# tuplex/tuplex

Measured on AMD Instinct MI355X. Metric: rows/s, higher is better.
Workload: dtype u8; 1 GPU; zillow-Z1 csv->map/withColumn/filter->tocsv (BASELINE.json configs[1]); mb_per_gpu=1024, sink=csv-device-resident

## Files before the change

### tuplex_amd/csrc/tpx_ci.hip.h

```cpp

#define TPX_CI_BYTES 4096
#define TPX_CI_RF_OFF 0
#define TPX_CI_BAD_OFF 136
#define TPX_CI_ENT_OFF 264
#define TPX_CI_CAP ((TPX_CI_BYTES - TPX_CI_ENT_OFF) / 4)
#define TPX_CI_NONE 0xFFFFu

__device__ __forceinline__ unsigned tpx_ci_zero32(unsigned x) {
    return ~(x | ((x | 0x80808080u) - 0x01010101u)) & 0x80808080u;
}

__device__ __forceinline__ unsigned tpx_ci_pack4(unsigned h) {
    unsigned x = h >> 7;
    x |= x >> 7;
    x |= x >> 14;
    return x & 0xFu;
}

struct tpx_ci_cls { unsigned q, s, n, r, h; };

__device__ __forceinline__ void tpx_ci_classify(unsigned w0, unsigned w1,
                                                unsigned w2, unsigned w3,
                                                char delim, unsigned valid,
                                                tpx_ci_cls* c) {
    const unsigned one = 0x01010101u;
    unsigned pq = one * (unsigned)'"', pd = one * (unsigned char)delim;
    unsigned pn = one * (unsigned)'\n', pr = one * (unsigned)'\r';
    unsigned w[4] = {w0, w1, w2, w3};
    unsigned q = 0, s = 0, n = 0, r = 0, h = 0;
    #pragma unroll
    for (int d = 0; d < 4; ++d) {
        unsigned v = w[d];
        unsigned zn = tpx_ci_zero32(v ^ pn);
        q |= tpx_ci_pack4(tpx_ci_zero32(v ^ pq)) << (4 * d);
        s |= tpx_ci_pack4(tpx_ci_zero32(v ^ pd) | zn) << (4 * d);
        n |= tpx_ci_pack4(zn) << (4 * d);
        r |= tpx_ci_pack4(tpx_ci_zero32(v ^ pr)) << (4 * d);
        h |= tpx_ci_pack4(v & 0x80808080u) << (4 * d);
    }
    c->q = q & valid; c->s = s & valid; c->n = n & valid;
    c->r = r & valid; c->h = h & valid;
}

__device__ __forceinline__ unsigned tpx_ci_inq(unsigned q16, unsigned par) {
    unsigned x = q16;
    x ^= x << 1; x ^= x << 2; x ^= x << 4; x ^= x << 8;
    x <<= 1;
    if (par) x = ~x;
    return x & 0xFFFFu;
}

__device__ __forceinline__ void tpx_ci_scatter(char* ci, int k, unsigned s16,
                                               unsigned n16, unsigned q16,
                                               unsigned ord, unsigned nl,
                                               unsigned qc0) {
    unsigned* ent = (unsigned*)(ci + TPX_CI_ENT_OFF);
    unsigned short* rf = (unsigned short*)(ci + TPX_CI_RF_OFF);
    while (s16) {
        int j = __ffs((int)s16) - 1;
        unsigned isnl = (n16 >> j) & 1u;
        unsigned qc = qc0 + (unsigned)__popc(q16 & ((1u << j) - 1u));
        if (ord < TPX_CI_CAP)
            ent[ord] = (unsigned)(k + j) | (isnl << 15) | (qc << 16);
        ++ord;
        if (isnl) {
            ++nl;
            if (nl <= 64 && ord <= TPX_CI_CAP) rf[nl] = (unsigned short)ord;
        }
        s16 &= s16 - 1;
    }
}

__device__ __forceinline__ int tpx_ci_row(const char* base, const char* ci,
                                          int r, int rs, int re, int rend,
                                          int span, int ncols, int* e0_out) {
    const unsigned* ent = (const unsigned*)(ci + TPX_CI_ENT_OFF);
    const unsigned short* rf = (const unsigned short*)(ci + TPX_CI_RF_OFF);
    const unsigned long long* bad =
        (const unsigned long long*)(ci + TPX_CI_BAD_OFF);
    if (re <= rs) return 0;
    unsigned e0 = rf[r], e1 = rf[r + 1];
    if (e0 == TPX_CI_NONE || e1 == TPX_CI_NONE) return 0;
    if (e1 != e0 + (unsigned)ncols) return 0;
    unsigned q = 0;
    if (e0 == 0) {
        if (r != 0) return 0;
    } else {
        unsigned pe = ent[e0 - 1];
        if (!(pe & 0x8000u) || (int)(pe & 0x3FFFu) != rs - 1) return 0;
        q = pe >> 16;
    }
    unsigned le = ent[e1 - 1];
    int lp = (int)(le & 0x3FFFu);
    if (le & 0x8000u) {
        if (lp != re - 1) return 0;
    } else {
        if (lp != re || re != span) return 0;
    }
    int b0 = rs >> 4, b1 = (re - 1) >> 4;
    for (int w = b0 >> 6; w <= (b1 >> 6); ++w) {
        int lo = w == (b0 >> 6) ? (b0 & 63) : 0;
        int hi = w == (b1 >> 6) ? (b1 & 63) : 63;
        unsigned long long m = (~0ULL << lo) & (~0ULL >> (63 - hi));
        if (bad[w] & m) return 0;
    }
    int cs = rs;
    for (int k = 0; k < ncols; ++k) {
        unsigned e = ent[e0 + (unsigned)k];
        int ce = k == ncols - 1 ? rend : (int)(e & 0x3FFFu);
        unsigned nq = ((e >> 16) - q) & 0xFFFFu;
        if (nq && (nq != 2 || ce - cs < 2 || base[cs] != '"' ||
                   base[ce - 1] != '"'))
            return 0;
        q = e >> 16;
        cs = (int)(e & 0x3FFFu) + 1;
    }
    *e0_out = (int)e0;
    return 1;
}

__device__ __forceinline__ void tpx_ci_cell(const char* base, const char* ci,
                                            int e0, int k, int ncols, int rs,
                                            int rend, tpx_cell* c) {
    const unsigned* ent = (const unsigned*)(ci + TPX_CI_ENT_OFF);
    unsigned e = ent[e0 + k];
    int cs = rs;
    unsigned q = 0;
    if (e0 + k > 0) {
        unsigned pe = ent[e0 + k - 1];
        cs = (int)(pe & 0x3FFFu) + 1;
        q = pe >> 16;
    }
    int ce = k == ncols - 1 ? rend : (int)(e & 0x3FFFu);
    if (((e >> 16) - q) & 0xFFFFu) {
        c->p = base + cs + 1; c->n = ce - cs - 2; c->flags = 1 | 8;
    } else {
        c->p = base + cs; c->n = ce - cs; c->flags = 0;
    }
}

#ifndef TPX_HOST_TEST
__device__ __forceinline__ unsigned tpx_wave_exscan32(unsigned v, int lane) {
    unsigned x = v;
    for (int o = 1; o < 64; o <<= 1) {
        unsigned y = __shfl_up(x, o);
        if (lane >= o) x += y;
    }
    return x - v;
}

__device__ __forceinline__ bool tpx_ci_stage(char* wave_lds, char* ci,
                                             const char* src, int span, int lo,
                                             char delim, int lane) {
    unsigned* ent = (unsigned*)(ci + TPX_CI_ENT_OFF);
    unsigned short* rf = (unsigned short*)(ci + TPX_CI_RF_OFF);
    unsigned long long* bad = (unsigned long long*)(ci + TPX_CI_BAD_OFF);
    rf[lane + 1] = (unsigned short)TPX_CI_NONE;
    if (lane == 0) rf[0] = 0;
    unsigned car_ord = 0, car_nl = 0, car_q = 0;
    bool pend = false;
    unsigned long long below = (1ull << lane) - 1ull;
    int trip = 0;
    uint4 pre = make_uint4(0, 0, 0, 0);
    if (lane * 16 + 16 <= span) pre = *(const uint4*)(src + lane * 16);
    for (int kb = 0; kb < span; kb += 64 * 16, ++trip) {
        int k = kb + lane * 16;
        unsigned w0 = 0, w1 = 0, w2 = 0, w3 = 0;
        if (k + 16 <= span) {
            uint4 v = pre;
            if (k + 64 * 16 + 16 <= span)
                pre = *(const uint4*)(src + k + 64 * 16);
            *(uint4*)(wave_lds + k) = v;
            w0 = v.x; w1 = v.y; w2 = v.z; w3 = v.w;
        } else {
            unsigned long long a = 0, b = 0;
            for (int j = k; j < span; ++j) {
                unsigned char ch = (unsigned char)src[j];
                wave_lds[j] = (char)ch;
                int t = j - k;
                if (t < 8) a |= (unsigned long long)ch << (8 * t);
                else b |= (unsigned long long)ch << (8 * (t - 8));
            }
            w0 = (unsigned)a; w1 = (unsigned)(a >> 32);
            w2 = (unsigned)b; w3 = (unsigned)(b >> 32);
        }
        int nv = span - k; nv = nv < 0 ? 0 : (nv > 16 ? 16 : nv);
        int nl_ = lo - k; nl_ = nl_ < 0 ? 0 : (nl_ > 16 ? 16 : nl_);
        unsigned valid = ((1u << nv) - 1u) & ~((1u << nl_) - 1u);
        tpx_ci_cls c;
        tpx_ci_classify(w0, w1, w2, w3, delim, valid, &c);
        unsigned pq = (unsigned)__popc(c.q);
        unsigned long long oddm = __ballot(pq & 1u);
        unsigned par = (car_q ^ (unsigned)__popcll(oddm & below)) & 1u;
        unsigned inq = tpx_ci_inq(c.q, par);
        unsigned s16 = c.s & ~inq, n16 = c.n & ~inq;
        unsigned ps = (unsigned)__popc(s16), pn = (unsigned)__popc(n16);
        unsigned ex = tpx_wave_exscan32(ps | (pn << 11) | (pq << 22), lane);
        unsigned xs = ex & 0x7FFu, xn = (ex >> 11) & 0x7FFu, xq = ex >> 22;
        unsigned long long nlf = __ballot(n16 & 1u);
        unsigned nxt = lane < 63 ? (unsigned)((nlf >> (lane + 1)) & 1ull) : 0u;
        unsigned badr = c.r & ~((n16 >> 1) | (nxt << 15));
        bool mypend = lane == 63 && (badr & 0x8000u);
        if (lane == 63) badr &= 0x7FFFu;
        unsigned long long bw = __ballot(c.h != 0 || badr != 0);
        if (lane == 0) {
            if (pend && !(nlf & 1ull)) bad[trip - 1] |= 1ull << 63;
            bad[trip] = bw;
        }
        pend = __ballot(mypend) != 0;
        tpx_ci_scatter(ci, k, s16, n16, c.q, car_ord + xs, car_nl + xn,
                       car_q + xq);
        car_ord += (unsigned)__builtin_amdgcn_readlane((int)(xs + ps), 63);
        car_nl += (unsigned)__builtin_amdgcn_readlane((int)(xn + pn), 63);
        car_q += (unsigned)__builtin_amdgcn_readlane((int)(xq + pq), 63);
    }
    if (pend && lane == 0) bad[trip - 1] |= 1ull << 63;
    bool ok = car_ord < TPX_CI_CAP;
    if (ok && car_nl < 64 && lane == 0) {
        ent[car_ord] = (unsigned)span | (car_q << 16);
        rf[car_nl + 1] = (unsigned short)(car_ord + 1);
    }
    __builtin_amdgcn_wave_barrier();
    return ok;
}
#endif
```

### tuplex_amd/csrc/tpx_rt.hip.h

```cpp
#pragma once
#if !defined(__HIPCC_RTC__) && !defined(__HIPRTC__)
#include <hip/hip_runtime.h>
#endif

#define TPX_WAVE 64

#ifndef TPX_OUTLINE
#define TPX_OUTLINE 0
#endif
#if TPX_OUTLINE
#define TPX_COLD __attribute__((noinline))
#else
#define TPX_COLD __forceinline__
#endif
#if TPX_OUTLINE >= 2
#define TPX_SHARED __attribute__((noinline))
#else
#define TPX_SHARED __forceinline__
#endif
struct tpx_i64r { long long v; int ec; };
struct tpx_f64r { double v; int ec; };

#define EC_OK 0
#define EC_NCV 7
// ... 639 lines not shown
    const char* p = start;
    bool neg = false;
    if (*p == '-') { neg = true; ++p; }
    while (p < end && *p >= '0' && *p <= '9') {
        x = x * 10 + (unsigned long long)(*p - '0');
        ++p;
    }
    if (p != end) return EC_I64PARSE;
    *out = (long long)(neg ? 0ULL - x : x);
    return EC_OK;
}

__device__ __forceinline__ int tpx_fast_atod(const char* start, const char* end,
                                             double* out) {
    if (start == end) return EC_NULLERROR;
    const char* p = start;
    double sign = 1.0;
    if (p < end && *p == '-') { sign = -1.0; ++p; }
    else if (p < end && *p == '+') ++p;
    double value = 0.0;
    while (p < end && *p >= '0' && *p <= '9') { value = 10.0 * value + (*p - '0'); ++p; }
    if (p < end && *p == '.') {
        double pow10 = 10.0;
        ++p;
        while (p < end && *p >= '0' && *p <= '9') {
            value += (*p - '0') / pow10;
            pow10 *= 10.0;
            ++p;
        }
    }
    int frac = 0;
    double scale = 1.0;
    if (p < end && (*p == 'e' || *p == 'E')) {
        ++p;
        if (p < end && *p == '-') { frac = 1; ++p; }
        else if (p < end && *p == '+') ++p;
        unsigned int exponent = 0;
        while (p < end && *p >= '0' && *p <= '9') { exponent = exponent * 10 + (*p - '0'); ++p; }
        if (exponent > 308) exponent = 308;
        while (exponent >= 50) { scale *= 1e50; exponent -= 50; }
        while (exponent >= 8)  { scale *= 1e8;  exponent -= 8; }
        while (exponent > 0)   { scale *= 10.0; exponent -= 1; }
    }
    int nanmatch = 0, infmatch = 0;
    if (p == start) {
        const char* t = "nan";
        while (nanmatch < 3 && p < end &&
               (*p == t[nanmatch] || *p == t[nanmatch] - 32)) { ++p; ++nanmatch; }
    }
    if (p == start) {
        const char* t = "infinity";
        while (infmatch < 8 && p < end &&
               (*p == t[infmatch] || *p == t[infmatch] - 32)) { ++p; ++infmatch; }
    }
    if (p != end) return EC_F64PARSE;
    if (nanmatch == 3) { *out = __builtin_nan(""); return EC_OK; }
    if (infmatch == 3 || infmatch == 8) { *out = sign * __builtin_inf(); return EC_OK; }
    *out = sign * (frac ? (value / scale) : (value * scale));
    return EC_OK;
}

__device__ TPX_SHARED tpx_i64r tpx_trim_atoi64(const char* p, long long n) {
    const char* a = p;
    const char* b = p + n;
    while (a < b && tpx_is_pyws(*a)) ++a;
    while (b > a && tpx_is_pyws(*(b - 1))) --b;
    tpx_i64r r{0, 0};
    r.ec = tpx_fast_atoi64(a, b, &r.v);
    return r;
}

__device__ TPX_SHARED tpx_f64r tpx_trim_atod(const char* p, long long n) {
    const char* a = p;
    const char* b = p + n;
    while (a < b && tpx_is_pyws(*a)) ++a;
    while (b > a && tpx_is_pyws(*(b - 1))) --b;
    tpx_f64r r{0.0, 0};
    r.ec = tpx_fast_atod(a, b, &r.v);
    return r;
}

__device__ __forceinline__ long long tpx_int_str(const tstr s, int* ec) {
    tpx_i64r r = tpx_trim_atoi64(s.p, s.n);
    if (r.ec != EC_OK) *ec = EC_VALUEERROR;
    return r.v;
}

__device__ __forceinline__ double tpx_float_str(const tstr s, int* ec) {
    tpx_f64r r = tpx_trim_atod(s.p, s.n);
    if (r.ec != EC_OK) *ec = EC_VALUEERROR;
    return r.v;
}

__device__ __forceinline__ long long tpx_int_f64(double x, int* ec) {
    if (!(x >= -9.223372036854775808e18 && x < 9.223372036854775808e18)) {
        *ec = x == x ? EC_OVERFLOW : EC_VALUEERROR;
        return 0;
    }
    return (long long)x;
}


__device__ __forceinline__ long long tpx_i64_digits(long long v) {
    unsigned long long x = v < 0 ? (unsigned long long)(-(v + 1)) + 1 : (unsigned long long)v;
    long long d = 1;
    while (x >= 10) { x /= 10; ++d; }
    return d + (v < 0 ? 1 : 0);
}

__device__ __forceinline__ void tpx_i64_write(char* dst, long long v, long long len) {
    unsigned long long x = v < 0 ? (unsigned long long)(-(v + 1)) + 1 : (unsigned long long)v;
    long long i = len;
    do { dst[--i] = '0' + (char)(x % 10); x /= 10; } while (x);
    if (v < 0) dst[0] = '-';
}

__device__ __forceinline__ tstr tpx_str_i64(TpxHeap& h, long long v, int* ec) {
    long long len = tpx_i64_digits(v);
    char* d = tpx_alloc(h, len);
    if (!d) { *ec = EC_MEMORYERROR; return tstr{nullptr, 0}; }
    tpx_i64_write(d, v, len);
    return tstr{d, len};
}

__device__ __forceinline__ tstr tpx_fmt0d(TpxHeap& h, long long width, long long v, int* ec) {
    long long dl = tpx_i64_digits(v);
    long long len = dl < width ? width : dl;
    char* d = tpx_alloc(h, len);
    if (!d) { *ec = EC_MEMORYERROR; return tstr{nullptr, 0}; }
    long long pad = len - dl;
    for (long long i = 0; i < pad; ++i) d[i] = '0';
    tpx_i64_write(d + pad, v, dl);
    if (v < 0 && pad > 0) {
        d[pad] = '0';
        d[0] = '-';
    }
    return tstr{d, len};
}

__device__ __forceinline__ tstr tpx_str_bool(bool b) {
    return b ? tstr{"True", 4} : tstr{"False", 5};
}

__device__ __forceinline__ tstr tpx_str_none() { return tstr{"None", 4}; }


__device__ TPX_SHARED long long tpx_csv_quote_scan(const tstr s) {
    bool need = false;
    long long q = 0;
    long long i = 0;
    while (i < s.n && (((unsigned long long)(s.p + i)) & 7)) {
        char c = s.p[i];
        if (c == '"') { ++q; need = true; }
        else if (c == ',' || c == '\n' || c == '\r') need = true;
        ++i;
    }
    for (; i + 32 <= s.n; i += 32) {
        unsigned long long v0 = *(const unsigned long long*)(s.p + i);
        unsigned long long v1 = *(const unsigned long long*)(s.p + i + 8);
        unsigned long long v2 = *(const unsigned long long*)(s.p + i + 16);
        unsigned long long v3 = *(const unsigned long long*)(s.p + i + 24);
        unsigned long long hq =
            tpx_swar_zero(v0 ^ (TPX_SWAR_ONE * (unsigned long long)'"')) |
            tpx_swar_zero(v1 ^ (TPX_SWAR_ONE * (unsigned long long)'"')) >> 1 |
            tpx_swar_zero(v2 ^ (TPX_SWAR_ONE * (unsigned long long)'"')) >> 2 |
            tpx_swar_zero(v3 ^ (TPX_SWAR_ONE * (unsigned long long)'"')) >> 3;
        unsigned long long ho = 0;
        ho |= tpx_swar_zero(v0 ^ (TPX_SWAR_ONE * (unsigned long long)',')) |
              tpx_swar_zero(v0 ^ (TPX_SWAR_ONE * (unsigned long long)'\n')) |
              tpx_swar_zero(v0 ^ (TPX_SWAR_ONE * (unsigned long long)'\r'));
        ho |= tpx_swar_zero(v1 ^ (TPX_SWAR_ONE * (unsigned long long)',')) |
              tpx_swar_zero(v1 ^ (TPX_SWAR_ONE * (unsigned long long)'\n')) |
              tpx_swar_zero(v1 ^ (TPX_SWAR_ONE * (unsigned long long)'\r'));
        ho |= tpx_swar_zero(v2 ^ (TPX_SWAR_ONE * (unsigned long long)',')) |
              tpx_swar_zero(v2 ^ (TPX_SWAR_ONE * (unsigned long long)'\n')) |
              tpx_swar_zero(v2 ^ (TPX_SWAR_ONE * (unsigned long long)'\r'));
        ho |= tpx_swar_zero(v3 ^ (TPX_SWAR_ONE * (unsigned long long)',')) |
              tpx_swar_zero(v3 ^ (TPX_SWAR_ONE * (unsigned long long)'\n')) |
              tpx_swar_zero(v3 ^ (TPX_SWAR_ONE * (unsigned long long)'\r'));
        if (hq) { q += __builtin_popcountll(hq); need = true; }
        if (ho) need = true;
    }
    for (; i + 8 <= s.n; i += 8) {
        unsigned long long v = *(const unsigned long long*)(s.p + i);
        unsigned long long hq =
            tpx_swar_zero(v ^ (TPX_SWAR_ONE * (unsigned long long)'"'));
        unsigned long long ho =
            tpx_swar_zero(v ^ (TPX_SWAR_ONE * (unsigned long long)',')) |
            tpx_swar_zero(v ^ (TPX_SWAR_ONE * (unsigned long long)'\n')) |
            tpx_swar_zero(v ^ (TPX_SWAR_ONE * (unsigned long long)'\r'));
        if (hq) { q += __builtin_popcountll(hq); need = true; }
        if (ho) need = true;
    }
    for (; i < s.n; ++i) {
        char c = s.p[i];
        if (c == '"') { ++q; need = true; }
        else if (c == ',' || c == '\n' || c == '\r') need = true;
    }
    return need ? q : -1;
}

__device__ __forceinline__ bool tpx_csv_needs_quote(const tstr s, long long* nquotes) {
    long long q = tpx_csv_quote_scan(s);
    *nquotes = q < 0 ? 0 : q;
    return q >= 0;
}

__device__ __forceinline__ long long tpx_csv_cell_len(const tstr s) {
    long long q;
    return tpx_csv_needs_quote(s, &q) ? s.n + q + 2 : s.n;
}

__device__ TPX_COLD char* tpx_csv_cell_write(char* w, const tstr s) {
    long long q;
    if (tpx_csv_needs_quote(s, &q)) {
        *w++ = '"';
        for (long long i = 0; i < s.n; ++i) {
            char c = s.p[i];
            *w++ = c;
            if (c == '"') *w++ = '"';
        }
        *w++ = '"';
    } else {
        tpx_memcpy(w, s.p, s.n);
        w += s.n;
    }
    return w;
}


struct tpx_f64n { unsigned long long N; int rc; bool neg; };

__device__ __forceinline__ int tpx_f64_csv_n_(double v, unsigned long long* N,
                                              bool* neg) {
    unsigned long long bits = (unsigned long long)__double_as_longlong(v);
    *neg = (bits >> 63) != 0;
    int exp = (int)((bits >> 52) & 0x7FF);
    unsigned long long man = bits & ((1ULL << 52) - 1);
    if (exp == 0x7FF) return 7;
    unsigned long long m;
    int e;
    if (exp == 0) { m = man; e = -1074; }
    else { m = man | (1ULL << 52); e = exp - 1075; }
    unsigned __int128 M = (unsigned __int128)m * 15625u;
    int k = e + 6;
    if (k >= 0) {
        if (k >= 62) return 7;
        unsigned __int128 S = M << k;
        if ((unsigned long long)(S >> 63)) return 7;
        *N = (unsigned long long)S;
        return 0;
    }
    k = -k;
    if (k >= 69) { *N = 0; return 0; }
    unsigned __int128 Nw = M >> k;
    unsigned __int128 rem = M & (((unsigned __int128)1 << k) - 1);
    unsigned __int128 half = (unsigned __int128)1 << (k - 1);
    if (rem > half || (rem == half && ((unsigned long long)Nw & 1))) ++Nw;
    if ((unsigned long long)(Nw >> 63)) return 7;
    *N = (unsigned long long)Nw;
    return 0;
}

__device__ TPX_SHARED tpx_f64n tpx_f64_csv_n_v(double v) {
    tpx_f64n r{0, 0, false};
    r.rc = tpx_f64_csv_n_(v, &r.N, &r.neg);
    return r;
}

__device__ __forceinline__ int tpx_f64_csv_n(double v, unsigned long long* N,
                                             bool* neg) {
    tpx_f64n r = tpx_f64_csv_n_v(v);
    if (r.rc == 0) *N = r.N;
    *neg = r.neg;
    return r.rc;
}

__device__ __forceinline__ long long tpx_f64_csv_len(unsigned long long N,
                                                     bool neg) {
    int d = 1;
    unsigned long long t = N;
    while (t >= 10) { t /= 10; ++d; }
    if (d < 7) d = 7;
    return (neg ? 1 : 0) + d + 1;
}

__device__ TPX_SHARED char* tpx_f64_csv_write(char* w,
                                            unsigned long long N,
                                            bool neg) {
    char buf[21];
    int nd = 0;
    unsigned long long t = N;
    do { buf[nd++] = (char)('0' + (t % 10)); t /= 10; } while (t);
    while (nd < 7) buf[nd++] = '0';
    if (neg) *w++ = '-';
    for (int i = nd - 1; i >= 6; --i) *w++ = buf[i];
    *w++ = '.';
    for (int i = 5; i >= 0; --i) *w++ = buf[i];
    return w;
}


#define TPX_CSV_CHUNK 4096
#define TPX_CSV_LANE_BYTES 64

#ifndef TPX_HOST_TEST
__device__ __forceinline__ long long tpx_wave_exscan(long long v) {
    long long x = v;
    for (int o = 1; o < 64; o <<= 1) {
        long long y = __shfl_up((long long)x, o);
        if ((threadIdx.x & 63) >= o) x += y;
    }
    return x - v;
}

__device__ __forceinline__ long long tpx_wave_sum(long long v) {
    for (int o = 32; o; o >>= 1) v += __shfl_down((long long)v, o);
    return __shfl((long long)v, 0);
}

struct TpxCsvSink {
    char* text;
    unsigned long long* cursor;
    unsigned long long cap;
    long long* b_off;
    long long* b_rows;
    long long* b_bytes;
    unsigned long long* rmeta;
};

__device__ __forceinline__ char* tpx_wave_commit_csv(const TpxCsvSink& K,
                                                     long long wb, bool kept,
                                                     long long sz,
                                                     long long* off_out,
                                                     long long* tot_out) {
    int lane = threadIdx.x & 63;
    long long v = kept ? sz : 0;
    long long off = tpx_wave_exscan(v);
    long long tot = tpx_wave_sum(v);
    unsigned long long m = __ballot(kept);
    int rank = __popcll(m & ((1ull << lane) - 1ull));
    unsigned long long base = 0;
    if (lane == 0) {
        unsigned long long need = ((unsigned long long)tot + 7ull) & ~7ull;
        if (need) base = atomicAdd(K.cursor, need);
        bool fits = base + need <= K.cap;
        K.b_off[wb] = fits ? (long long)base : 0;
        K.b_rows[wb] = fits ? (long long)__popcll(m) : 0;
        K.b_bytes[wb] = fits ? tot : 0;
        if (!fits) base = ~0ull;
    }
    base = __shfl((unsigned long long)base, 0);
    *off_out = off;
    *tot_out = tot;
    if (base == ~0ull || tot == 0) return nullptr;
    if (kept)
        K.rmeta[wb * 64 + rank] =
            ((unsigned long long)lane << 32) | (unsigned long long)off;
    return K.text + base;
}

__device__ __forceinline__ void tpx_scan64(const char* __restrict__ data,
                                           long long a, long long b,
                                           int quotes_on,
                                           long long* lq, long long* l0,
                                           long long* l1) {
    long long qq = 0, e0 = 0, e1 = 0;
    if (b - a == TPX_CSV_LANE_BYTES && ((a & 15) == 0)) {
        #pragma unroll
        for (int v = 0; v < 4; ++v) {
            uint4 w = *(const uint4*)(data + a + v * 16);
            unsigned words[4] = {w.x, w.y, w.z, w.w};
            #pragma unroll
            for (int k = 0; k < 4; ++k)
                #pragma unroll
                for (int s = 0; s < 4; ++s) {
                    unsigned ch = (words[k] >> (8 * s)) & 0xFF;
                    if (quotes_on && ch == '"') ++qq;
                    else if (ch == '\n') { if (qq & 1) ++e1; else ++e0; }
                }
        }
    } else {
        for (long long i = a; i < b; ++i) {
            char ch = data[i];
            if (quotes_on && ch == '"') ++qq;
            else if (ch == '\n') { if (qq & 1) ++e1; else ++e0; }
        }
    }
    *lq = qq; *l0 = e0; *l1 = e1;
}

extern "C" __global__ void tpx_csv_chunk_stats(const char* __restrict__ data,
                                               long long size, long long nchunks,
                                               long long* __restrict__ q,
                                               long long* __restrict__ c0,
                                               long long* __restrict__ c1,
                                               int quotes_on) {
    int lane = threadIdx.x & 63;
    int wid = threadIdx.x >> 6;
    int wpb = blockDim.x >> 6;
    long long wstride = (long long)gridDim.x * wpb;
    for (long long c = (long long)blockIdx.x * wpb + wid; c < nchunks;
         c += wstride) {
        long long a = c * TPX_CSV_CHUNK + (long long)lane * TPX_CSV_LANE_BYTES;
        long long b = a + TPX_CSV_LANE_BYTES;
        if (a > size) a = size;
        if (b > size) b = size;
        long long lq, l0, l1;
        tpx_scan64(data, a, b, quotes_on, &lq, &l0, &l1);
        long long pref = tpx_wave_exscan(lq);
        bool odd = (pref & 1) != 0;
        long long tot_q = tpx_wave_sum(lq);
        long long tot0 = tpx_wave_sum(odd ? l1 : l0);
        long long tot1 = tpx_wave_sum(odd ? l0 : l1);
        if (lane == 0) { q[c] = tot_q; c0[c] = tot0; c1[c] = tot1; }
    }
}

extern "C" __global__ void tpx_csv_select_counts(const long long* __restrict__ qscan,
                                                 const long long* __restrict__ c0,
                                                 const long long* __restrict__ c1,
                                                 long long* __restrict__ rc,
                                                 long long nchunks) {
    long long stride = (long long)gridDim.x * blockDim.x;
    for (long long c = (long long)blockIdx.x * blockDim.x + threadIdx.x;
         c < nchunks; c += stride)
        rc[c] = (qscan[c] & 1) ? c1[c] : c0[c];
}

extern "C" __global__ void tpx_csv_emit_rows(const char* __restrict__ data,
                                             long long size, long long nchunks,
                                             const long long* __restrict__ qscan,
                                             const long long* __restrict__ base,
                                             long long* __restrict__ row_offs,
                                             int quotes_on, long long row_lo,
                                             long long row_hi) {
    int lane = threadIdx.x & 63;
    int wid = threadIdx.x >> 6;
    int wpb = blockDim.x >> 6;
    long long wstride = (long long)gridDim.x * wpb;
    if (blockIdx.x == 0 && threadIdx.x == 0 && row_lo == 0) row_offs[0] = 0;
    for (long long c = (long long)blockIdx.x * wpb + wid; c < nchunks;
         c += wstride) {
        if (base[c] >= row_hi) continue;
        if (c + 1 < nchunks && base[c + 1] < row_lo) continue;
        long long a = c * TPX_CSV_CHUNK + (long long)lane * TPX_CSV_LANE_BYTES;
        long long b = a + TPX_CSV_LANE_BYTES;
        if (a > size) a = size;
        if (b > size) b = size;
        long long lq, l0, l1;
        tpx_scan64(data, a, b, quotes_on, &lq, &l0, &l1);
        long long pref_q = tpx_wave_exscan(lq);
        long long start_par = (qscan[c] + pref_q) & 1;
        long long sel = start_par ? l1 : l0;
        long long lane_base = base[c] + tpx_wave_exscan(sel);
        long long qq = 0, idx = lane_base;
        if (b - a == TPX_CSV_LANE_BYTES && ((a & 15) == 0)) {
            #pragma unroll
            for (int v = 0; v < 4; ++v) {
                uint4 w = *(const uint4*)(data + a + v * 16);
                unsigned words[4] = {w.x, w.y, w.z, w.w};
                #pragma unroll
                for (int k = 0; k < 4; ++k)
                    #pragma unroll
                    for (int s2 = 0; s2 < 4; ++s2) {
                        unsigned ch = (words[k] >> (8 * s2)) & 0xFF;
                        if (quotes_on && ch == '"') ++qq;
                        else if (ch == '\n' && (((qq + start_par) & 1) == 0))
                            row_offs[1 + idx++] = a + v * 16 + k * 4 + s2 + 1;
                    }
            }
        } else {
            for (long long i = a; i < b; ++i) {
                char ch = data[i];
                if (quotes_on && ch == '"') ++qq;
                else if (ch == '\n' && (((qq + start_par) & 1) == 0))
                    row_offs[1 + idx++] = i + 1;
            }
        }
    }
}

#endif

struct tpx_cell { const char* p; long long n; int flags; };

__device__ __forceinline__ long long tpx_memchr_hi_spec(
        const char* p, long long n, char c, unsigned long long* hi,
        int chk_comma, int* spec) {
    unsigned long long pat = TPX_SWAR_ONE * (unsigned char)c;
    unsigned long long sp_acc = 0;
    long long i = 0;
    #define TPX_SPECW(v) \
        (tpx_swar_zero((v) ^ (TPX_SWAR_ONE * (unsigned long long)'"')) | \
         tpx_swar_zero((v) ^ (TPX_SWAR_ONE * (unsigned long long)'\r')) | \
         (chk_comma ? tpx_swar_zero((v) ^ (TPX_SWAR_ONE * (unsigned long long)',')) : 0ULL))
    #define TPX_SPECB(ch) \
        ((ch) == '"' || (ch) == '\r' || (chk_comma && (ch) == ','))
    while (i < n && (((unsigned long long)(p + i)) & 7)) {
        unsigned char ch = p[i];
        *hi |= ch & 0x80u;
        if ((char)ch == c) { if (sp_acc) *spec = 1; return i; }
        if (TPX_SPECB(ch)) sp_acc = 1;
        ++i;
    }
    for (; i + 32 <= n; i += 32) {
        unsigned long long v0 = *(const unsigned long long*)(p + i);
        unsigned long long v1 = *(const unsigned long long*)(p + i + 8);
        unsigned long long v2 = *(const unsigned long long*)(p + i + 16);
        unsigned long long v3 = *(const unsigned long long*)(p + i + 24);
        unsigned long long h0 = tpx_swar_zero(v0 ^ pat);
        unsigned long long h1 = tpx_swar_zero(v1 ^ pat);
        unsigned long long h2 = tpx_swar_zero(v2 ^ pat);
        unsigned long long h3 = tpx_swar_zero(v3 ^ pat);
        if (h0 | h1 | h2 | h3) {
            unsigned long long hw, hv, sw;
            long long base;
            if (h0) { hw = h0; hv = v0; sw = TPX_SPECW(v0); base = i; }
            else if (h1) { hw = h1; hv = v1; sw = TPX_SPECW(v1); base = i + 8;
                           sp_acc |= TPX_SPECW(v0);
                           *hi |= v0 & TPX_SWAR_HIGH; }
            else if (h2) { hw = h2; hv = v2; sw = TPX_SPECW(v2); base = i + 16;
                           sp_acc |= TPX_SPECW(v0) | TPX_SPECW(v1);
                           *hi |= (v0 | v1) & TPX_SWAR_HIGH; }
            else { hw = h3; hv = v3; sw = TPX_SPECW(v3); base = i + 24;
                   sp_acc |= TPX_SPECW(v0) | TPX_SPECW(v1) | TPX_SPECW(v2);
                   *hi |= (v0 | v1 | v2) & TPX_SWAR_HIGH; }
            long long b = (__ffsll((long long)hw) - 1) / 8;
            *hi |= hv & TPX_SWAR_HIGH & TPX_SWAR_UPTO(b);
            sp_acc |= sw & ((b ? (1ULL << (8 * b)) : 1ULL) - 1);
            if (sp_acc) *spec = 1;
            return base + b;
        }
        sp_acc |= TPX_SPECW(v0) | TPX_SPECW(v1) | TPX_SPECW(v2) | TPX_SPECW(v3);
        *hi |= (v0 | v1 | v2 | v3) & TPX_SWAR_HIGH;
    }
    for (; i + 8 <= n; i += 8) {
        unsigned long long v = *(const unsigned long long*)(p + i);
        unsigned long long hit = tpx_swar_zero(v ^ pat);
        if (hit) {
            long long b = (__ffsll((long long)hit) - 1) / 8;
            *hi |= v & TPX_SWAR_HIGH & TPX_SWAR_UPTO(b);
            sp_acc |= TPX_SPECW(v) & ((b ? (1ULL << (8 * b)) : 1ULL) - 1);
            if (sp_acc) *spec = 1;
            return i + b;
        }
        *hi |= v & TPX_SWAR_HIGH;
        sp_acc |= TPX_SPECW(v);
    }
    for (; i < n; ++i) {
        unsigned char ch = p[i];
        *hi |= ch & 0x80u;
        if ((char)ch == c) { if (sp_acc) *spec = 1; return i; }
        if (TPX_SPECB(ch)) sp_acc = 1;
    }
    if (sp_acc) *spec = 1;
    return -1;
    #undef TPX_SPECW
    #undef TPX_SPECB
}

__device__ __forceinline__ const char* tpx_csv_next_cell(const char* p,
                                                         const char* end,
                                                         tpx_cell* c, bool* more,
                                                         char delim,
                                                         unsigned long long* hi) {
    c->flags = 0;
    *more = false;
    if (p < end && *p == '"') {
        const char* s = p + 1;
        const char* q = s;
        bool esc = false;
        while (q < end) {
            long long k = tpx_memchr_hi(q, end - q, '"', hi);
            if (k < 0) { q = end; break; }
            q += k;
            if (q + 1 < end && q[1] == '"') { esc = true; q += 2; continue; }
            break;
        }
        if (q >= end) { c->p = p; c->n = end - p; c->flags = 4; return end; }
        c->p = s; c->n = q - s; c->flags = 1 | (esc ? 2 : 0) | 8;
        ++q;
        if (q < end && *q != delim) c->flags |= 4;
        long long kd = tpx_memchr_hi(q, end - q, delim, hi);
        q = kd < 0 ? end : q + kd;
        if (q < end) { *more = true; ++q; }
        return q;
    }
    int spec = 0;
    long long kd = tpx_memchr_hi_spec(p, end - p, delim, hi,
                                      delim != ',', &spec);
    const char* q = kd < 0 ? end : p + kd;
    c->p = p; c->n = q - p;
    if (spec) c->flags |= 8;
    if (q < end) { *more = true; ++q; }
    return q;
}


struct tpx_grp { unsigned long long q, d, s; };

struct tpx_mwalk {
    const char* ab;
    int off, endb;
    int g;
    int pos;
    bool more;
    tpx_grp G;
    unsigned long long hib;
};

__device__ __forceinline__ unsigned long long tpx_mm8(unsigned long long h) {
    return ((h >> 7) * 0x0102040810204080ULL) >> 56;
}

__device__ __forceinline__ void tpx_mw_group(tpx_mwalk& S, int g, char delim,
                                             int chk_comma) {
    const unsigned long long* w =
        (const unsigned long long*)(S.ab + ((long long)g << 6));
    unsigned long long pq = TPX_SWAR_ONE * (unsigned long long)'"';
    unsigned long long pd = TPX_SWAR_ONE * (unsigned char)delim;
    unsigned long long pr = TPX_SWAR_ONE * (unsigned long long)'\r';
    unsigned long long pc = TPX_SWAR_ONE * (unsigned long long)',';
    unsigned long long q = 0, d = 0, s = 0, h = 0;
    #pragma unroll
    for (int k = 0; k < 8; ++k) {
        unsigned long long v = w[k];
        q |= tpx_mm8(tpx_swar_zero(v ^ pq)) << (8 * k);
        d |= tpx_mm8(tpx_swar_zero(v ^ pd)) << (8 * k);
        unsigned long long sv = tpx_swar_zero(v ^ pr);
        if (chk_comma) sv |= tpx_swar_zero(v ^ pc);
        s |= tpx_mm8(sv) << (8 * k);
        h |= tpx_mm8(v & TPX_SWAR_HIGH) << (8 * k);
    }
    int base = g << 6;
    int lo = S.off - base; if (lo < 0) lo = 0;
    int hi = S.endb - base; if (hi > 64) hi = 64;
    unsigned long long rm = (hi <= lo) ? 0ULL :
        ((hi >= 64 ? ~0ULL : ((1ULL << hi) - 1)) & ~((1ULL << lo) - 1));
    S.G.q = q & rm;
    S.G.d = d & rm;
    S.G.s = (s | q) & rm;
    S.hib |= h & rm;
    S.g = g;
}

__device__ __forceinline__ void tpx_mw_init(tpx_mwalk& S, const char* rp,
                                            const char* rend) {
    S.ab = (const char*)((unsigned long long)rp & ~7ULL);
    S.off = (int)(rp - S.ab);
    S.endb = S.off + (int)(rend - rp);
    S.g = -1;
    S.pos = S.off;
    S.more = true;
    S.hib = 0;
}

__device__ __forceinline__ int tpx_mw_test_q(tpx_mwalk& S, int k, char delim,
                                             int chk) {
    if (k >= S.endb) return 0;
    if ((k >> 6) != S.g) tpx_mw_group(S, k >> 6, delim, chk);
    return (int)((S.G.q >> (k & 63)) & 1);
}

__device__ __forceinline__ int tpx_mw_test_d(tpx_mwalk& S, int k, char delim,
                                             int chk) {
    if (k >= S.endb) return 0;
    if ((k >> 6) != S.g) tpx_mw_group(S, k >> 6, delim, chk);
    return (int)((S.G.d >> (k & 63)) & 1);
}

__device__ __forceinline__ int tpx_mw_next_d(tpx_mwalk& S, int k, char delim,
                                             int chk, int* spec) {
    unsigned long long sp_acc = 0;
    for (;;) {
        if (k >= S.endb) { if (sp_acc) *spec = 1; return S.endb; }
        if ((k >> 6) != S.g) tpx_mw_group(S, k >> 6, delim, chk);
        int local = k & 63;
        unsigned long long ge = local ? (~0ULL << local) : ~0ULL;
        unsigned long long d = S.G.d & ge;
        unsigned long long s = S.G.s & ge;
        if (d) {
            int b = __ffsll((long long)d) - 1;
            sp_acc |= s & ((b ? (1ULL << b) : 1ULL) - 1);
            if (sp_acc) *spec = 1;
            return (S.g << 6) + b;
        }
        sp_acc |= s;
        k = (S.g + 1) << 6;
    }
}

__device__ __forceinline__ int tpx_mw_next_q(tpx_mwalk& S, int k, char delim,
                                             int chk) {
    for (;;) {
        if (k >= S.endb) return S.endb;
        if ((k >> 6) != S.g) tpx_mw_group(S, k >> 6, delim, chk);
        int local = k & 63;
        unsigned long long ge = local ? (~0ULL << local) : ~0ULL;
        unsigned long long q = S.G.q & ge;
        if (q) return (S.g << 6) + (__ffsll((long long)q) - 1);
        k = (S.g + 1) << 6;
    }
}

__device__ __forceinline__ void tpx_mw_cell(tpx_mwalk& S, tpx_cell* c,
                                            char delim, int chk) {
    c->flags = 0;
    S.more = false;
    int pos = S.pos;
    if (pos < S.endb && tpx_mw_test_q(S, pos, delim, chk)) {
        int q = pos + 1;
        bool esc = false;
        for (;;) {
            int cq = tpx_mw_next_q(S, q, delim, chk);
            if (cq >= S.endb) {
                c->p = S.ab + pos; c->n = S.endb - pos; c->flags = 4;
                S.pos = S.endb;
                return;
            }
            if (cq + 1 < S.endb && tpx_mw_test_q(S, cq + 1, delim, chk)) {
                esc = true; q = cq + 2; continue;
            }
            q = cq;
            break;
        }
        c->p = S.ab + pos + 1; c->n = q - (pos + 1);
        c->flags = 1 | (esc ? 2 : 0) | 8;
        ++q;
        if (q < S.endb && !tpx_mw_test_d(S, q, delim, chk)) c->flags |= 4;
        int spec = 0;
        int nd = tpx_mw_next_d(S, q, delim, chk, &spec);
        if (nd < S.endb) { S.more = true; S.pos = nd + 1; } else S.pos = S.endb;
        return;
    }
    int spec = 0;
    int nd = tpx_mw_next_d(S, pos, delim, chk, &spec);
    c->p = S.ab + pos; c->n = nd - pos;
    if (spec) c->flags |= 8;
    if (nd < S.endb) { S.more = true; S.pos = nd + 1; } else S.pos = S.endb;
}

template <int NC>
struct tpx_rowcells {
    int off[NC];
    int n[NC];
    unsigned long long flags;
    int ncells;
    int badf;
    bool more;
    bool hib;
};

template <int NC, char DELIM, int CHK>
__device__ TPX_COLD tpx_rowcells<NC> tpx_walk_row(const char* rp,
                                                  const char* rend) {
    static_assert(NC <= 16, "4 flag bits per cell in 64");
    tpx_rowcells<NC> R;
    tpx_mwalk S;
    tpx_mw_init(S, rp, rend);
    R.flags = 0;
    R.ncells = 0;
    R.badf = 0;
    bool avail = true;
    #pragma unroll 1
    for (int k = 0; k < NC; ++k) {
        R.off[k] = 0;
        R.n[k] = 0;
        if (!avail) continue;
        tpx_cell c;
        tpx_mw_cell(S, &c, DELIM, CHK);
        avail = S.more;
        R.off[k] = (int)(c.p - rp);
        R.n[k] = (int)c.n;
        R.flags |= (unsigned long long)(c.flags & 15) << (4 * k);
        R.badf |= c.flags;
        R.ncells = k + 1;
    }
    R.more = avail;
    R.hib = S.hib != 0;
    return R;
// ... 526 lines not shown
```

Before: 978.4 million rows/s.

## Rewrite CSV chunk stats and row emission with SWAR bitsets and coalesced loads

Replaces the per-byte scalar scan over 64-byte lane slices in the chunk-stats and row-emit kernels with SWAR bitmask detection of quotes and newlines. The data is loaded as coalesced 16-byte strided words, quote parity is carried across lanes with ballot and mbcnt, and row offsets are emitted from bitmasks. The emit kernel now has each wave ballot over 64 candidate chunks to skip ones outside the row range, and it uses a cheap ballot path when no lane has more than one row. Shared bit helpers move into the runtime header. This adds complexity, and the 16-bit packing of the even/odd counts assumes each chunk has fewer than 65536 newlines.

```diff
diff --git a/tuplex_amd/csrc/tpx_ci.hip.h b/tuplex_amd/csrc/tpx_ci.hip.h
--- a/tuplex_amd/csrc/tpx_ci.hip.h
+++ b/tuplex_amd/csrc/tpx_ci.hip.h
@@ -5,17 +5,6 @@
 #define TPX_CI_ENT_OFF 264
 #define TPX_CI_CAP ((TPX_CI_BYTES - TPX_CI_ENT_OFF) / 4)
 #define TPX_CI_NONE 0xFFFFu
-
-__device__ __forceinline__ unsigned tpx_ci_zero32(unsigned x) {
-    return ~(x | ((x | 0x80808080u) - 0x01010101u)) & 0x80808080u;
-}
-
-__device__ __forceinline__ unsigned tpx_ci_pack4(unsigned h) {
-    unsigned x = h >> 7;
-    x |= x >> 7;
-    x |= x >> 14;
-    return x & 0xFu;
-}
 
 struct tpx_ci_cls { unsigned q, s, n, r, h; };
 
@@ -31,23 +20,19 @@
     #pragma unroll
     for (int d = 0; d < 4; ++d) {
         unsigned v = w[d];
-        unsigned zn = tpx_ci_zero32(v ^ pn);
-        q |= tpx_ci_pack4(tpx_ci_zero32(v ^ pq)) << (4 * d);
-        s |= tpx_ci_pack4(tpx_ci_zero32(v ^ pd) | zn) << (4 * d);
-        n |= tpx_ci_pack4(zn) << (4 * d);
-        r |= tpx_ci_pack4(tpx_ci_zero32(v ^ pr)) << (4 * d);
-        h |= tpx_ci_pack4(v & 0x80808080u) << (4 * d);
+        unsigned zn = tpx_bs_zero32(v ^ pn);
+        q |= tpx_bs_pack4(tpx_bs_zero32(v ^ pq)) << (4 * d);
+        s |= tpx_bs_pack4(tpx_bs_zero32(v ^ pd) | zn) << (4 * d);
+        n |= tpx_bs_pack4(zn) << (4 * d);
+        r |= tpx_bs_pack4(tpx_bs_zero32(v ^ pr)) << (4 * d);
+        h |= tpx_bs_pack4(v & 0x80808080u) << (4 * d);
     }
     c->q = q & valid; c->s = s & valid; c->n = n & valid;
     c->r = r & valid; c->h = h & valid;
 }
 
 __device__ __forceinline__ unsigned tpx_ci_inq(unsigned q16, unsigned par) {
-    unsigned x = q16;
-    x ^= x << 1; x ^= x << 2; x ^= x << 4; x ^= x << 8;
-    x <<= 1;
-    if (par) x = ~x;
-    return x & 0xFFFFu;
+    return tpx_bs_inq(q16, par);
 }
 
 __device__ __forceinline__ void tpx_ci_scatter(char* ci, int k, unsigned s16,
@@ -140,15 +125,6 @@
 }
 
 #ifndef TPX_HOST_TEST
-__device__ __forceinline__ unsigned tpx_wave_exscan32(unsigned v, int lane) {
-    unsigned x = v;
-    for (int o = 1; o < 64; o <<= 1) {
-        unsigned y = __shfl_up(x, o);
-        if (lane >= o) x += y;
-    }
-    return x - v;
-}
-
 __device__ __forceinline__ bool tpx_ci_stage(char* wave_lds, char* ci,
                                              const char* src, int span, int lo,
                                              char delim, int lane) {
diff --git a/tuplex_amd/csrc/tpx_rt.hip.h b/tuplex_amd/csrc/tpx_rt.hip.h
--- a/tuplex_amd/csrc/tpx_rt.hip.h
+++ b/tuplex_amd/csrc/tpx_rt.hip.h
@@ -965,7 +965,84 @@
 
 
 #define TPX_CSV_CHUNK 4096
-#define TPX_CSV_LANE_BYTES 64
+
+
+__device__ __forceinline__ unsigned tpx_bs_zero32(unsigned x) {
+    return ~(x | ((x | 0x80808080u) - 0x01010101u)) & 0x80808080u;
+}
+
+__device__ __forceinline__ unsigned tpx_bs_pack4(unsigned h) {
+    unsigned x = h >> 7;
+    x |= x >> 7;
+    x |= x >> 14;
+    return x & 0xFu;
+}
+
+__device__ __forceinline__ unsigned tpx_bs_inq(unsigned q16, unsigned par) {
+    unsigned x = q16;
+    x ^= x << 1; x ^= x << 2; x ^= x << 4; x ^= x << 8;
+    x <<= 1;
+    if (par) x = ~x;
+    return x & 0xFFFFu;
+}
+
+struct tpx_bs_det { unsigned q[4], n[4], mq, mn; };
+
+__device__ __forceinline__ void tpx_bs_detect(unsigned w0, unsigned w1,
+                                              unsigned w2, unsigned w3,
+                                              int quotes_on, tpx_bs_det* d) {
+    const unsigned pq = 0x01010101u * (unsigned)'"';
+    const unsigned pn = 0x01010101u * (unsigned)'\n';
+    unsigned w[4] = {w0, w1, w2, w3};
+    #pragma unroll
+    for (int i = 0; i < 4; ++i) {
+        d->n[i] = tpx_bs_zero32(w[i] ^ pn);
+        d->q[i] = quotes_on ? tpx_bs_zero32(w[i] ^ pq) : 0u;
+    }
+    d->mn = d->n[0] | d->n[1] >> 1 | d->n[2] >> 2 | d->n[3] >> 3;
+    d->mq = d->q[0] | d->q[1] >> 1 | d->q[2] >> 2 | d->q[3] >> 3;
+}
+
+__device__ __forceinline__ unsigned tpx_bs_pos16(const unsigned h[4]) {
+    return tpx_bs_pack4(h[0]) | tpx_bs_pack4(h[1]) << 4 |
+           tpx_bs_pack4(h[2]) << 8 | tpx_bs_pack4(h[3]) << 12;
+}
+
+__device__ __forceinline__ void tpx_bs_count16(unsigned w0, unsigned w1,
+                                               unsigned w2, unsigned w3,
+                                               int quotes_on, unsigned* nq,
+                                               unsigned* e, unsigned* o) {
+    tpx_bs_det d;
+    tpx_bs_detect(w0, w1, w2, w3, quotes_on, &d);
+    unsigned nn = (unsigned)__builtin_popcount(d.mn), od = 0;
+    if (d.mq && d.mn)
+        od = (unsigned)__builtin_popcount(tpx_bs_pos16(d.n) &
+                              tpx_bs_inq(tpx_bs_pos16(d.q), 0u));
+    *nq = (unsigned)__builtin_popcount(d.mq);
+    *e = nn - od;
+    *o = od;
+}
+
+__device__ __forceinline__ unsigned tpx_bs_rows16(const tpx_bs_det* d,
+                                                  unsigned par) {
+    if (!d->mn) return 0u;
+    unsigned n16 = tpx_bs_pos16(d->n);
+    if (!d->mq) return par ? 0u : n16;
+    return n16 & ~tpx_bs_inq(tpx_bs_pos16(d->q), par);
+}
+
+__device__ __forceinline__ void tpx_bs_load_tail(const char* data, long long k,
+                                                 long long size, unsigned w[4]) {
+    unsigned long long a = 0, b = 0;
+    for (long long j = k; j < size && j < k + 16; ++j) {
+        unsigned long long ch = (unsigned char)data[j];
+        int t = (int)(j - k);
+        if (t < 8) a |= ch << (8 * t);
+        else b |= ch << (8 * (t - 8));
+    }
+    w[0] = (unsigned)a; w[1] = (unsigned)(a >> 32);
+    w[2] = (unsigned)b; w[3] = (unsigned)(b >> 32);
+}
 
 #ifndef TPX_HOST_TEST
 __device__ __forceinline__ long long tpx_wave_exscan(long long v) {
@@ -980,6 +1057,25 @@
 __device__ __forceinline__ long long tpx_wave_sum(long long v) {
     for (int o = 32; o; o >>= 1) v += __shfl_down((long long)v, o);
     return __shfl((long long)v, 0);
+}
+
+__device__ __forceinline__ unsigned tpx_wave_exscan32(unsigned v, int lane) {
+    unsigned x = v;
+    for (int o = 1; o < 64; o <<= 1) {
+        unsigned y = __shfl_up(x, o);
+        if (lane >= o) x += y;
+    }
+    return x - v;
+}
+
+__device__ __forceinline__ unsigned tpx_wave_sum32(unsigned v) {
+    for (int o = 32; o; o >>= 1) v += __shfl_xor(v, o);
+    return v;
+}
+
+__device__ __forceinline__ unsigned tpx_lanes_below(unsigned long long m) {
+    return __builtin_amdgcn_mbcnt_hi((unsigned)(m >> 32),
+               __builtin_amdgcn_mbcnt_lo((unsigned)m, 0u));
 }
 
 struct TpxCsvSink {
@@ -1023,34 +1119,26 @@
     return K.text + base;
 }
 
-__device__ __forceinline__ void tpx_scan64(const char* __restrict__ data,
-                                           long long a, long long b,
-                                           int quotes_on,
-                                           long long* lq, long long* l0,
-                                           long long* l1) {
-    long long qq = 0, e0 = 0, e1 = 0;
-    if (b - a == TPX_CSV_LANE_BYTES && ((a & 15) == 0)) {
+__device__ __forceinline__ void tpx_bs_load_chunk(const char* __restrict__ data,
+                                                  long long cb, long long size,
+                                                  int lane, uint4 v[4]) {
+    if (cb + TPX_CSV_CHUNK <= size) {
         #pragma unroll
-        for (int v = 0; v < 4; ++v) {
-            uint4 w = *(const uint4*)(data + a + v * 16);
-            unsigned words[4] = {w.x, w.y, w.z, w.w};
-            #pragma unroll
-            for (int k = 0; k < 4; ++k)
-                #pragma unroll
-                for (int s = 0; s < 4; ++s) {
-                    unsigned ch = (words[k] >> (8 * s)) & 0xFF;
-                    if (quotes_on && ch == '"') ++qq;
-                    else if (ch == '\n') { if (qq & 1) ++e1; else ++e0; }
-                }
-        }
+        for (int t = 0; t < 4; ++t)
+            v[t] = *(const uint4*)(data + cb + t * 1024 + lane * 16);
     } else {
-        for (long long i = a; i < b; ++i) {
-            char ch = data[i];
-            if (quotes_on && ch == '"') ++qq;
-            else if (ch == '\n') { if (qq & 1) ++e1; else ++e0; }
-        }
-    }
-    *lq = qq; *l0 = e0; *l1 = e1;
+        #pragma unroll
+        for (int t = 0; t < 4; ++t) {
+            long long k = cb + t * 1024 + lane * 16;
+            if (k + 16 <= size) {
+                v[t] = *(const uint4*)(data + k);
+            } else {
+                unsigned w[4];
+                tpx_bs_load_tail(data, k, size, w);
+                v[t] = make_uint4(w[0], w[1], w[2], w[3]);
+            }
+        }
+    }
 }
 
 extern "C" __global__ void tpx_csv_chunk_stats(const char* __restrict__ data,
@@ -1065,18 +1153,27 @@
     long long wstride = (long long)gridDim.x * wpb;
     for (long long c = (long long)blockIdx.x * wpb + wid; c < nchunks;
          c += wstride) {
-        long long a = c * TPX_CSV_CHUNK + (long long)lane * TPX_CSV_LANE_BYTES;
-        long long b = a + TPX_CSV_LANE_BYTES;
-        if (a > size) a = size;
-        if (b > size) b = size;
-        long long lq, l0, l1;
-        tpx_scan64(data, a, b, quotes_on, &lq, &l0, &l1);
-        long long pref = tpx_wave_exscan(lq);
-        bool odd = (pref & 1) != 0;
-        long long tot_q = tpx_wave_sum(lq);
-        long long tot0 = tpx_wave_sum(odd ? l1 : l0);
-        long long tot1 = tpx_wave_sum(odd ? l0 : l1);
-        if (lane == 0) { q[c] = tot_q; c0[c] = tot0; c1[c] = tot1; }
+        uint4 v[4];
+        tpx_bs_load_chunk(data, c * TPX_CSV_CHUNK, size, lane, v);
+        unsigned carry = 0;
+        unsigned acc = 0, accq = 0;
+        #pragma unroll
+        for (int t = 0; t < 4; ++t) {
+            unsigned nq, e, o;
+            tpx_bs_count16(v[t].x, v[t].y, v[t].z, v[t].w, quotes_on, &nq, &e,
+                           &o);
+            unsigned long long odd = __ballot(nq & 1u);
+            unsigned par = (carry ^ tpx_lanes_below(odd)) & 1u;
+            acc += par ? (o | e << 16) : (e | o << 16);
+            accq += nq;
+            carry ^= (unsigned)__popcll(odd);
+        }
+        unsigned s = tpx_wave_sum32(acc), sq = tpx_wave_sum32(accq);
+        if (lane == 0) {
+            q[c] = (long long)sq;
+            c0[c] = (long long)(s & 0xFFFFu);
+            c1[c] = (long long)(s >> 16);
+        }
     }
 }
 
@@ -1089,6 +1186,44 @@
     for (long long c = (long long)blockIdx.x * blockDim.x + threadIdx.x;
          c < nchunks; c += stride)
         rc[c] = (qscan[c] & 1) ? c1[c] : c0[c];
+}
+
+__device__ __forceinline__ void tpx_bs_emit_chunk(const char* __restrict__ data,
+                                                  long long size, long long c,
+                                                  unsigned par0, long long rbase,
+                                                  long long* __restrict__ row_offs,
+                                                  int quotes_on, int lane) {
+    long long cb = c * TPX_CSV_CHUNK;
+    uint4 v[4];
+    tpx_bs_load_chunk(data, cb, size, lane, v);
+    unsigned carry = par0 & 1u;
+    long long run = rbase;
+    #pragma unroll
+    for (int t = 0; t < 4; ++t) {
+        tpx_bs_det d;
+        tpx_bs_detect(v[t].x, v[t].y, v[t].z, v[t].w, quotes_on, &d);
+        unsigned long long odd = __ballot(__popc(d.mq) & 1);
+        unsigned par = (carry ^ tpx_lanes_below(odd)) & 1u;
+        carry ^= (unsigned)__popcll(odd) & 1u;
+        unsigned r16 = tpx_bs_rows16(&d, par);
+        unsigned cnt = (unsigned)__popc(r16);
+        unsigned ex, tot;
+        if (__ballot(cnt > 1u) == 0) {
+            unsigned long long one = __ballot(cnt != 0u);
+            ex = tpx_lanes_below(one);
+            tot = (unsigned)__popcll(one);
+        } else {
+            ex = tpx_wave_exscan32(cnt, lane);
+            tot = (unsigned)__builtin_amdgcn_readlane((int)(ex + cnt), 63);
+        }
+        long long idx = run + ex;
+        long long k = cb + t * 1024 + lane * 16;
+        while (r16) {
+            row_offs[1 + idx++] = k + __ffs((int)r16);
+            r16 &= r16 - 1;
+        }
+        run += tot;
+    }
 }
 
 extern "C" __global__ void tpx_csv_emit_rows(const char* __restrict__ data,
@@ -1103,43 +1238,20 @@
     int wpb = blockDim.x >> 6;
     long long wstride = (long long)gridDim.x * wpb;
     if (blockIdx.x == 0 && threadIdx.x == 0 && row_lo == 0) row_offs[0] = 0;
-    for (long long c = (long long)blockIdx.x * wpb + wid; c < nchunks;
-         c += wstride) {
-        if (base[c] >= row_hi) continue;
-        if (c + 1 < nchunks && base[c + 1] < row_lo) continue;
-        long long a = c * TPX_CSV_CHUNK + (long long)lane * TPX_CSV_LANE_BYTES;
-        long long b = a + TPX_CSV_LANE_BYTES;
-        if (a > size) a = size;
-        if (b > size) b = size;
-        long long lq, l0, l1;
-        tpx_scan64(data, a, b, quotes_on, &lq, &l0, &l1);
-        long long pref_q = tpx_wave_exscan(lq);
-        long long start_par = (qscan[c] + pref_q) & 1;
-        long long sel = start_par ? l1 : l0;
-        long long lane_base = base[c] + tpx_wave_exscan(sel);
-        long long qq = 0, idx = lane_base;
-        if (b - a == TPX_CSV_LANE_BYTES && ((a & 15) == 0)) {
-            #pragma unroll
-            for (int v = 0; v < 4; ++v) {
-                uint4 w = *(const uint4*)(data + a + v * 16);
-                unsigned words[4] = {w.x, w.y, w.z, w.w};
-                #pragma unroll
-                for (int k = 0; k < 4; ++k)
-                    #pragma unroll
-                    for (int s2 = 0; s2 < 4; ++s2) {
-                        unsigned ch = (words[k] >> (8 * s2)) & 0xFF;
-                        if (quotes_on && ch == '"') ++qq;
-                        else if (ch == '\n' && (((qq + start_par) & 1) == 0))
-                            row_offs[1 + idx++] = a + v * 16 + k * 4 + s2 + 1;
-                    }
-            }
-        } else {
-            for (long long i = a; i < b; ++i) {
-                char ch = data[i];
-                if (quotes_on && ch == '"') ++qq;
-                else if (ch == '\n' && (((qq + start_par) & 1) == 0))
-                    row_offs[1 + idx++] = i + 1;
-            }
+    for (long long cg = (long long)blockIdx.x * wpb + wid; cg < nchunks;
+         cg += 64 * wstride) {
+        long long mc = cg + lane * wstride;
+        bool want = false;
+        if (mc < nchunks)
+            want = base[mc] < row_hi &&
+                   !(mc + 1 < nchunks && base[mc + 1] < row_lo);
+        unsigned long long todo = __ballot(want);
+        while (todo) {
+            int i = __ffsll((long long)todo) - 1;
+            todo &= todo - 1;
+            long long c = cg + i * wstride;
+            tpx_bs_emit_chunk(data, size, c, (unsigned)qscan[c] & 1u, base[c],
+                              row_offs, quotes_on, lane);
         }
     }
 }
```

New measurement: 1.055 billion rows/s, median of 6. 1.08x the previous value.
